# s-a-malik/fumi

Hardware: AMD Instinct MI355X
Metric: episodes/sec (5-way 5-shot FuMI) (higher is better)
Workload: dtype f32; 1 GPU; FuMI 5-way 5-shot, 32 query/class, ResNet-152-style 2048-d embeddings, im_hid [256,64], GloVe-300 token text (L=128, V=20000, mean pool), text_hid 256, 1 inner step, second-order meta-gradient + Adam step; BASELINE.json configs[1]; episodes_per_gpu=32, global_meta_batch=32, parallelism=episode-sharded x1, 1 all-reduce of the flat gradient

## Files before the change

### fumi_amd/csrc/common.h

```cpp
#pragma once
#include <hip/hip_runtime.h>
#include <stdint.h>
#include <stddef.h>
#include <vector>
#include "../../include/fumi_hip.h"

typedef float f32x4 __attribute__((ext_vector_type(4)));
typedef float f32x16 __attribute__((ext_vector_type(16)));

struct f32pair { float x, y; };
struct ProfRec { int phase; hipEvent_t a, b; };
struct fumi_ws {
    int device;
    char* base;
    size_t cap;
    size_t off;
    int* status;
    int* status_host;
    const float* pub_src; float* pub_dst; int pub_n; unsigned long long pub_seq;
    struct AdamPending* adam;
    struct GlovePending* glove;
    float* text_grad;
    int* acnt;
    int* hcnt;
// ... 498 lines not shown
    if (tid < parts * N) {
        const int part = tid / N, n = tid - part * N;
        float s0 = 0.f, s1 = 0.f;
        int m = part;
        for (; m + parts < M; m += 2 * parts) { s0 += X[(long)m * ld + n]; s1 += X[(long)(m + parts) * ld + n]; }
        if (m < M) s0 += X[(long)m * ld + n];
        lds[part * N + n] = s0 + s1;
    }
    __syncthreads();
    for (int n = tid; n < N; n += nt) {
        float s = 0.f;
        for (int pp = 0; pp < parts; ++pp) s += lds[pp * N + n];
        f(n, s);
    }
}
__host__ __device__ __forceinline__ int wg_ld(int cols) { return ((cols + 31) & ~31) + 4; }

__device__ __forceinline__ void wg_stage_tab_to_lds(StageTab* Tl, int ntab = 1, int kernarg_bytes = 0) {
    const int* src = (const int*)__builtin_amdgcn_kernarg_segment_ptr();
    int* dst = (int*)Tl;
    for (int i = threadIdx.x; i < ntab * (int)(sizeof(StageTab) / 4); i += blockDim.x) dst[i] = src[i];
    if (kernarg_bytes > 0) {
        const int first = ntab * (int)sizeof(StageTab) / 64, last = (kernarg_bytes + 63) / 64;
        const int ln = first + (int)threadIdx.x;
        if (ln < last) {
            int dummy;
            asm volatile("global_load_dword %0, %1, off" : "=v"(dummy) : "v"((const char*)src + (long)ln * 64) : "memory");
            asm volatile("s_waitcnt vmcnt(0)" ::: "memory");
            asm volatile("" :: "v"(dummy));
        }
    }
// ... 257 lines not shown
```

### fumi_amd/csrc/episode.hip

```cpp
#include "common.h"
#include <algorithm>
#include <stdlib.h>

namespace {

unsigned long long* g_epi_trace = nullptr;
int g_spin_limit = 1 << 22;
constexpr int QR = 32;
constexpr int MAXL = FUMI_MAX_HIDDEN;

struct EpiBuf {
    float *A0, *G;
    float *D, *cs;
    float *bcur[MAXL], *bh;
    float *Wslot[MAXL], *Whslot;
    float *ta[MAXL], *tdz[MAXL], *tp, *te;
    float *lg;
    float *aq[MAXL], *zq[MAXL], *lbar, *qcs;
    float *pW[MAXL], *pb[MAXL], *pWh, *pbh, *pb0, *pD, *ploss, *pcorr;
    float *Wb[MAXL], *bb[MAXL], *Whb, *bhb, *b0b, *Db;
    float *abar[MAXL], *X0, *X1, *eb, *lb;
    float *A0bar;
    float *A0bar_q; int ldsr, ldq;
    float *apart; int *acnt;
// ... 23 lines not shown
    return drop_mix(h + 0xC2B2AE35U * (unsigned)layer);
}
__device__ __forceinline__ float drop_relu(const EpiDims& d, unsigned key, long idx, float z) {
    if (z <= 0.f) return 0.f;
    if (d.drop_thr == 0) return z;
    return drop_mix(key ^ (unsigned)idx) >= d.drop_thr ? z * d.mscale : 0.f;
}
__device__ __forceinline__ f32x4 drop_relu4(const EpiDims& d, unsigned key, long idx, const f32x4& z) {
    f32x4 o;
#pragma unroll
    for (int e = 0; e < 4; ++e) o[e] = drop_relu(d, key, idx + e, z[e]);
    return o;
}
constexpr int QUERY_CALL = 1 << 20;

struct EpiParams {
    const float* W[MAXL];
    const float* b[MAXL];
};

__device__ __forceinline__ int label(const int64_t* y, long i, int N, int* status) {
    long v = y[i];
    if (v < 0 || v >= N) { atomicOr(status, FUMI_ST_LABEL_RANGE); v = 0; }
    return (int)v;
}

__global__ __launch_bounds__(512) void adapt_kernel(EpiDims d, EpiBuf w, EpiParams prm, const int64_t* y_s,
                                                     const float* head, int* status) {
    extern __shared__ __attribute__((aligned(16))) float sm[];
    const int sm_cap = w.lds_adapt;
// ... 103 lines not shown
            wg_mm2(sm, sm_cap, hi, hp, S, dz(i), 1, hi, a(i - 1), hp, 1, [&](int m, int n) { return Wci[(long)m * hp + n]; },
                   [&](int m, int n, float acc, float pre) { Wni[(long)m * hp + n] = pre - alpha * acc; });
            float* bi = w.bcur[i] + (long)b * hi;
            wg_colsum(sm, sm_cap, S, hi, dz(i), hi, [&](int n, float s) { bi[n] -= alpha * s; });
        }
        if (L == 1) __syncthreads();
        {
            wg_ew((long)S * h0, D, D, dz(0), nullptr, [&](long, float x, float y, float) { return x + y; });
        }
        __syncthreads(); STAMP()
    }
    wg_colsum(sm, sm_cap, S, h0, D, h0, [&](int n, float s) { cs[n] = s; });
#undef STAMP
}

__host__ __device__ inline int q_r4(int x) { return (x + 3) & ~3; }
__host__ __device__ inline int q_r16(int x) { return (x + 15) & ~15; }
constexpr int ALDS_CAP = 40000;
struct ALay { int a[MAXL], dz[MAXL], W[MAXL], bi[MAXL], Wh, G, D, e, cs, bh, total; };
__host__ __device__ inline void adapt_layout(ALay& y, int L, const int* h, int S, int N) {
    int off = 0;
    const int RS = q_r4(S);
    for (int i = 0; i < MAXL; ++i) { y.a[i] = y.dz[i] = y.W[i] = y.bi[i] = 0; }
    for (int i = 0; i < L; ++i) { y.a[i] = off; off += RS * wg_ld(h[i]); }
    for (int i = 1; i < L; ++i) { y.dz[i] = off; off += RS * wg_ld(h[i]); }
    y.G = off; off += RS * wg_ld(S);
    y.e = off; off += RS * wg_ld(N);
    y.D = off; off += RS * wg_ld(h[0]);
    for (int i = 1; i < L; ++i) { y.W[i] = off; off += q_r16(h[i]) * wg_ld(h[i - 1]); y.bi[i] = off; off += q_r4(h[i]); }
    y.Wh = off; off += q_r16(N) * wg_ld(h[L - 1]);
    y.cs = off; off += q_r4(h[0]);
    y.bh = off; off += q_r4(N);
// ... 371 lines not shown
               [&](int m, int n, float acc, float pre) { zp[(long)m * hp + n] = pre > 0.f ? acc * d.mscale : 0.f; });
        __syncthreads();
    }
    float* A0bq = w.A0bar_q + ((long)b * w.ldq + r0) * h0;
    wg_copy(A0bq, z(0), (long)nr * h0);
    float* pb0 = w.pb0 + pt * h0;
    wg_colsum(sm, sm_cap, nr, h0, z(0), h0, [&](int n, float s) { pb0[n] = s; });
    __syncthreads();
    float* pD = w.pD + pt * (long)S * h0;
    wg_mm2(sm, sm_cap, S, h0, nr, Gqs, 1, S, z(0), h0, 1, [&](int m, int n) { return pb0[n]; },
           [&](int m, int n, float acc, float pre) { pD[(long)m * h0 + n] = -alpha * (acc + pre); });
}

constexpr int QLDS_CAP = 40000;
struct QLay { int a[MAXL], W[MAXL], bi[MAXL], Wh, Wh2, Gq, D, lq, b0, cs, pb0, bh, total; };
__host__ __device__ inline void query_layout(QLay& y, int L, const int* h, int S, int N, bool fused = false) {
    int off = 0;
    for (int i = 0; i < MAXL; ++i) { y.a[i] = y.W[i] = y.bi[i] = 0; }
    for (int i = 0; i < L; ++i) { y.a[i] = off; off += QR * wg_ld(h[i]); }
    for (int i = 1; i < L; ++i) { y.W[i] = off; off += q_r16(h[i]) * wg_ld(h[i - 1]); y.bi[i] = off; off += q_r4(h[i]); }
    y.Wh = off; off += q_r16(N) * wg_ld(h[L - 1]);
    y.Wh2 = off; if (fused) off += q_r16(N) * wg_ld(h[L - 1]);
    y.Gq = off; off += QR * wg_ld(S);
    y.D = off; off += q_r4(S) * wg_ld(h[0]);
    y.lq = off; off += QR * wg_ld(N);
    y.b0 = off; off += q_r4(h[0]);
    y.cs = off; off += q_r4(h[0]);
    y.pb0 = off; off += q_r4(h[0]);
    y.bh = off; off += q_r4(N);
    y.total = off;
}

template <bool FUSED>
__global__ __launch_bounds__(512) void query_lds_kernel(StageTab stg, StageTab stg_sup, EpiDims d, EpiBuf w, QLay y, const int64_t* y_q,
                                                        float* logits_q, int64_t* preds_q, float* preds_f, int* status,
                                                        const int64_t* y_s) {
    extern __shared__ __attribute__((aligned(16))) float sm[];
    __shared__ float s_loss[QR];
    __shared__ float s_corr[QR];
    __shared__ StageTab s_stg2[2];
    __shared__ int s_lab[QR];
    StageTab& s_stg = s_stg2[0];
    const int tile = blockIdx.x, b = blockIdx.y, tid = threadIdx.x, nt = blockDim.x;
    int qi = 0;
#define QSTAMP() if (w.trace && tid == 0 && blockIdx.x == 0 && blockIdx.y == 0) w.trace[64 + qi++] = __builtin_amdgcn_s_memrealtime();
    QSTAMP()
    const int S = d.S, N = d.N, L = d.L, H = d.H, h0 = d.h[0], Qn = d.Qn;
    const int r0 = tile * QR, nr = min(QR, Qn - r0);
    const float alpha = d.alpha;
    const int ldq = wg_ld(N), ldG = wg_ld(S), ld0 = wg_ld(h0), ldH = wg_ld(H);
    auto a = [&](int i) { return sm + y.a[i]; };
    auto lda = [&](int i) { return wg_ld(d.h[i]); };

    const int my_label = tid < nr ? label(y_q + (long)b * Qn + r0, tid, N, status) : 0;
    const int my_label_s = (FUSED && tid < S) ? label(y_s + (long)b * S, tid, N, status) : 0;
    if (FUSED && tid < S && tid < QR) s_lab[tid] = my_label_s;
    wg_stage_tab_to_lds(s_stg2, 2, (int)(2 * sizeof(StageTab) + sizeof(EpiDims) + sizeof(EpiBuf) + sizeof(QLay) + 64));
    for (int i = tid * 4, tot = y.total; i < tot; i += nt * 4) *(f32x4*)(sm + i) = (f32x4){0.f, 0.f, 0.f, 0.f};
    __syncthreads(); QSTAMP()
    int whq = y.Wh;
    if constexpr (FUSED) {
        const int nt_ = (Qn + QR - 1) / QR;
        const bool lead = tile == 0 && d.taped;
        const bool lead_w = tile == (nt_ > 1 ? 1 : 0) && d.taped, lead_r = tile == (nt_ > 2 ? 2 : 0) && d.taped;
        const f32x4 z4s = {0.f, 0.f, 0.f, 0.f};
        f32x4 qv[4]; bool qok[4];
        {
            const float* A0q = w.A0 + ((long)b * (S + Qn) + S + r0) * h0;
            const int c4n = h0 >> 2;
#pragma unroll
            for (int i = 0; i < 4; ++i) {
                const int f = tid + 512 * i, m = f / c4n, n = (f - m * c4n) << 2;
                qok[i] = m < nr;
                qv[i] = *(const f32x4*)(A0q + (long)(qok[i] ? m : 0) * h0 + (qok[i] ? n : 0));
            }
        }
        wg_stage_rows<20>(&s_stg2[1], b, tile, 0, nr, sm);
        wg_lds_barrier();
        float* a0 = a(0); float* a1 = a(1); float* W1 = sm + y.W[1]; float* b1 = sm + y.bi[1];
        float* Wh = sm + y.Wh; float* Wh2 = sm + y.Wh2; float* bh = sm + y.bh; float* Dl = sm + y.D; float* csl = sm + y.cs;
        const float* b0l = sm + y.b0; float* e_ = sm + y.lq;
        const int h1 = d.h[1], ld1 = wg_ld(h1);
        const long tp = (long)b * w.ntape;
        auto store_img = [&](float* dst, long drs, const float* img, int ld, int rows, int cols) {
            const int c4n = (cols + 3) >> 2;
            for (int i = tid; i < rows * c4n; i += nt) {
                const int r = i / c4n, cc = (i - r * c4n) << 2;
                wg_st4(dst + (long)r * drs + cc, *(const f32x4*)(img + r * ld + cc), min(4, cols - cc));
            }
        };
        if (lead_w) {
            store_img(w.Wslot[1] + (long)b * w.nslot * ((long)h1 * h0), h0, W1, ld0, h1, h0);
            store_img(w.Whslot + (long)b * w.nslot * N * H, H, Wh, ldH, N, H);
        }
        {
            const unsigned key0 = drop_key(d, b, 0, 0);
            float* ta0 = w.ta[0] + tp * S * h0;
// ... 98 lines not shown
        wg_lds_barrier(); QSTAMP()
    }

    {
        float* a0 = a(0);
        const float* b0l = sm + y.b0; const float* csl = sm + y.cs;
        const unsigned keyq0 = drop_key(d, b, QUERY_CALL, 0);
        wg_lmm_wide<true>(nr, h0, S, sm + y.Gq, ldG, sm + y.D, ld0, [&](int m, int n, const f32x4& acc, int, auto) {
            float* p = a0 + m * ld0 + n;
            const f32x4 pre = *(const f32x4*)p + (*(const f32x4*)(b0l + n) - alpha * *(const f32x4*)(csl + n));
            *(f32x4*)p = drop_relu4(d, keyq0, (long)(r0 + m) * h0 + n, pre - alpha * acc);
        });
    }
    wg_lds_barrier(); QSTAMP()
    for (int i = 1; i < L; ++i) {
        const int hi = d.h[i], hp = d.h[i - 1];
        float* ai = a(i); const int ldi = lda(i);
        const float* bi = sm + y.bi[i];
        const unsigned keyqi = drop_key(d, b, QUERY_CALL, i);
        wg_lmm<true, true>(nr, hi, hp, a(i - 1), lda(i - 1), sm + y.W[i], wg_ld(hp), [&](int m, int n, const f32x4& acc, int) {
            *(f32x4*)(ai + m * ldi + n) = drop_relu4(d, keyqi, (long)(r0 + m) * hi + n, acc + *(const f32x4*)(bi + n));
        });
        wg_lds_barrier(); QSTAMP()
    }
    float* lq = sm + y.lq;
    {
        float* lg = logits_q + ((long)b * Qn + r0) * N;
        const float* bhl = sm + y.bh;
        wg_lmm<true, true>(nr, N, H, a(L - 1), ldH, sm + whq, ldH, [&](int m, int n, const f32x4& acc, int cnt) {
            const f32x4 v = acc + *(const f32x4*)(bhl + n);
            *(f32x4*)(lq + m * ldq + n) = v;
// ... 41 lines not shown
            wg_st4(pWh + m * H + n, acc, cnt);
        });
        float* pbh = w.pbh + pt * N;
        wg_lcolsum(nr, N, lbar, ldq, [&](int n, float s) { pbh[n] = s; });
    }
    wg_lds_barrier(); QSTAMP()
    {
        float* zl = a(L - 1);
        wg_lmm_wide<true>(nr, H, N, lbar, ldq, sm + whq, ldH, [&](int m, int n, const f32x4& acc, int, auto) {
            float* p = zl + m * ldH + n;
            *(f32x4*)p = relu_bwd4(*(const f32x4*)p, acc);
        });
    }
    wg_lds_barrier(); QSTAMP()
    for (int i = L - 1; i >= 1; --i) {
        const int hi = d.h[i], hp = d.h[i - 1];
        const float* zi = a(i); const int ldi = lda(i), ldp = lda(i - 1);
        float* pWi = w.pW[i] + pt * (long)hi * hp;
        wg_lmm_wide<false>(hi, hp, nr, zi, ldi, a(i - 1), ldp, [&](int m, int n, const f32x4& acc, int cnt, auto) {
            wg_st4(pWi + (long)m * hp + n, acc, cnt);
        });
        float* pbi = w.pb[i] + pt * hi;
        wg_lcolsum(nr, hi, zi, ldi, [&](int n, float s) { pbi[n] = s; });
        wg_lds_barrier(); QSTAMP()
        float* zp = a(i - 1);
        wg_lmm_wide<true>(nr, hp, hi, zi, ldi, sm + y.W[i], wg_ld(hp), [&](int m, int n, const f32x4& acc, int, auto) {
            float* p = zp + m * ldp + n;
            *(f32x4*)p = relu_bwd4(*(const f32x4*)p, acc);
        });
        wg_lds_barrier(); QSTAMP()
    }
// ... 154 lines not shown
                   [&](int m, int n) { return f32pair{Db[(long)m * h0 + n], cs[n]}; },
                   [&](int m, int n, float acc, f32pair pre) { Db[(long)m * h0 + n] = pre.x - alpha * (acc + pre.y); });
            __syncthreads();
        }
    }
    float* hb = head_bar + (long)b * N * (H + 1);
    for (int j = tid; j < N * H; j += nt) hb[(j / H) * (H + 1) + (j % H)] = Whb[j];
    for (int j = tid; j < N; j += nt) hb[j * (H + 1) + H] = bhb[j];
}

constexpr int RLDS_CAP = 40000;
struct RLay {
    int Wb[MAXL], bb[MAXL], a[MAXL], dz[MAXL], W[MAXL], ab[MAXL];
    int Db, A0bs, b0b, Whb, bhb, Wh, p, e, eb, G, dab0, X0, X1, cs, ldX, total;
};
inline void reverse_layout(RLay& y, int L, const int* h, int S, int N, int P) {
    int off = 0;
    const int RS = q_r4(S), h0c = h[0] / P, H = h[L - 1];
    auto take = [&](int rows, int ld) { const int o = off; off += rows * ld; return o; };
    for (int i = 0; i < MAXL; ++i) y.Wb[i] = y.bb[i] = y.a[i] = y.dz[i] = y.W[i] = y.ab[i] = 0;
    int maxh1 = 4;
    for (int i = 1; i < L; ++i) maxh1 = h[i] > maxh1 ? h[i] : maxh1;
    y.ldX = wg_ld(maxh1);
    for (int i = 1; i < L; ++i) {
        const int kc = i == 1 ? h0c : h[i - 1];
        y.Wb[i] = take(q_r16(h[i]), wg_ld(kc)); y.W[i] = take(q_r16(h[i]), wg_ld(kc)); y.bb[i] = take(1, q_r4(h[i]));
        y.a[i] = take(RS, wg_ld(h[i])); y.dz[i] = take(RS, wg_ld(h[i])); y.ab[i] = take(RS, wg_ld(h[i]));
    }
    y.a[0] = take(RS, wg_ld(h0c)); y.ab[0] = take(RS, wg_ld(h0c)); y.dab0 = take(RS, wg_ld(h0c));
    y.Db = take(RS, wg_ld(h0c)); y.A0bs = take(RS, wg_ld(h0c));
    y.X0 = take(RS, y.ldX); y.X1 = take(RS, y.ldX);
    y.Whb = take(q_r16(N), wg_ld(H)); y.Wh = take(q_r16(N), wg_ld(H));
    y.p = take(RS, wg_ld(N)); y.e = take(RS, wg_ld(N)); y.eb = take(RS, wg_ld(N)); y.G = take(RS, wg_ld(S));
    y.b0b = take(1, q_r4(h0c)); y.cs = take(1, q_r4(h0c)); y.bhb = take(1, q_r4(N));
    y.total = off + 64;
}

__global__ __launch_bounds__(512) void reverse_lds_kernel(StageTab stg_init, StageTab stg_step, EpiDims d, EpiBuf w, RLay y,
                                                          int P, float* loss_b, float* acc_b, float* head_bar) {
    extern __shared__ __attribute__((aligned(16))) float sm[];
    __shared__ StageTab s_stg[2];
    const int tid = threadIdx.x, nt = blockDim.x;
    const int xcd = blockIdx.x & 7, jq = blockIdx.x >> 3;
    const int b = xcd + 8 * (jq / P), c = jq % P;
    if (b >= d.B) return;
    int ri = 0;
#define RSTAMP() if (w.trace && tid == 0 && blockIdx.x == 0) w.trace[128 + ri++] = __builtin_amdgcn_s_memrealtime();
    RSTAMP()
    const int S = d.S, N = d.N, L = d.L, H = d.H, h0 = d.h[0], h0c = h0 / P, c0 = c * h0c, h1 = d.h[1];
    const float alpha = d.alpha, ms = d.mscale;
    const int ntile = w.ntile;
    if (tid == 0 && c == 0) {
        float ls = 0.f, cr = 0.f;
        for (int t = 0; t < ntile; ++t) { ls += w.ploss[(long)b * ntile + t]; cr += w.pcorr[(long)b * ntile + t]; }
        loss_b[b] = ls / (float)d.Qn;
        acc_b[b] = cr / (float)d.Qn;
    }
    if (!d.need_grad) return;

    const int ldc = wg_ld(h0c), ldN = wg_ld(N), ldS = wg_ld(S), ldH = wg_ld(H), ldX = y.ldX;
    auto ldh = [&](int i) { return wg_ld(d.h[i]); };
    const f32x4 z4 = {0.f, 0.f, 0.f, 0.f};
    auto relu_bwd4 = [&](const f32x4& act, const f32x4& g) {
        f32x4 o;
#pragma unroll
        for (int e = 0; e < 4; ++e) o[e] = act[e] > 0.f ? g[e] * ms : 0.f;
        return o;
    };
    auto ew = [&](int cols, auto&& f) {
        const int c4n = (cols + 3) >> 2;
        for (int i = tid; i < S * c4n; i += nt) { const int m = i / c4n; f(m, (i - m * c4n) << 2); }
    };
    auto store_img = [&](float* dst, long drs, const float* img, int ld, int rows, int cols) {
        const int c4n = (cols + 3) >> 2;
        for (int i = tid; i < rows * c4n; i += nt) {
            const int r = i / c4n, cc = (i - r * c4n) << 2;
// ... 6 lines not shown
    __syncthreads(); RSTAMP()
    wg_stage_rows<3, 8>(&s_stg[0], b, 0, c, 0, sm);
    wg_lds_barrier(); RSTAMP()

    float* Wb1 = sm + y.Wb[1]; float* Db = sm + y.Db; float* A0bs = sm + y.A0bs; float* b0b = sm + y.b0b;
    float* Whb = sm + y.Whb; float* bhb = sm + y.bhb; float* cs = sm + y.cs;
    float* a0 = sm + y.a[0]; float* ab0 = sm + y.ab[0]; float* dab0 = sm + y.dab0; float* W1 = sm + y.W[1];
    float* Wh = sm + y.Wh; float* pp = sm + y.p; float* ee = sm + y.e; float* eb = sm + y.eb; float* G = sm + y.G;
    float* Xa = sm + y.X0; float* Xb = sm + y.X1;

    if (d.second_order) {
        for (int t = d.T - 1; t >= 0; --t) {
            const int round = d.T - 1 - t;
            wg_stage_rows<8, 1>(&s_stg[1], b, t, c, 0, sm);
            wg_lds_barrier(); RSTAMP()
            for (int i = 1; i < L; ++i) { float* abi = sm + y.ab[i]; const int ldi = ldh(i); ew(d.h[i], [&](int m, int n) { *(f32x4*)(abi + m * ldi + n) = z4; }); }
            ew(h0c, [&](int m, int n) {
                *(f32x4*)(ab0 + m * ldc + n) = z4;
                *(f32x4*)(dab0 + m * ldc + n) = relu_bwd4(*(const f32x4*)(a0 + m * ldc + n), *(const f32x4*)(Db + m * ldc + n));
            });
            wg_lds_barrier(); RSTAMP()
            const float* dz1 = sm + y.dz[1]; const int ld1 = ldh(1);
            wg_lmm<true, true>(S, h1, h0c, dab0, ldc, W1, ldc, [&](int m, int n, const f32x4& acc, int) { *(f32x4*)(Xa + m * ldX + n) = acc; });
            wg_lmm<true, true>(S, h1, h0c, a0, ldc, Wb1, ldc, [&](int m, int n, const f32x4& acc, int) {
                float* px = Xa + m * ldX + n; *(f32x4*)px = *(const f32x4*)px - alpha * acc;
            });
            wg_lmm_wide<true>(S, h0c, h1, dz1, ld1, Wb1, ldc, [&](int m, int n, const f32x4& acc, int, auto) {
                float* pa = ab0 + m * ldc + n; *(f32x4*)pa = *(const f32x4*)pa - alpha * acc;
            });
            wg_lds_barrier(); RSTAMP()
            float* xb = w.xpart + (((long)b * 2 + (round & 1)) * 8) * (long)S * h1;
// ... 30 lines not shown
                for (int i = tid; i < S * w4; i += nt) {
                    const int m = i / w4, n = i - m * w4;
                    float v = 0.f;
                    if (n < h1) {
                        if (P > 1) { for (int cc = 0; cc < P; ++cc) v += __hip_atomic_load(xb + (long)cc * S * h1 + m * h1 + n, __ATOMIC_RELAXED, __HIP_MEMORY_SCOPE_AGENT); }
                        else v = Xa[m * ldX + n];
                        v = a1[m * ld1 + n] > 0.f ? (v - alpha * bb1[n]) * ms : 0.f;
                    }
                    Xb[m * ldX + n] = v;
                }
            }
            wg_lds_barrier(); RSTAMP()
            int cur = 1;
            auto X = [&](int i) { return i ? Xb : Xa; };
            for (int i = 2; i < L; ++i) {
                const int hi = d.h[i], hp = d.h[i - 1], ldi = ldh(i), ldp = ldh(i - 1);
                const float* dab = X(cur); float* nxt = X(cur ^ 1);
                const float* bbi = sm + y.bb[i]; float* Wbi = sm + y.Wb[i]; const float* ai = sm + y.a[i];
                const float* dzi = sm + y.dz[i]; float* abp = sm + y.ab[i - 1];
                wg_lmm<true, true>(S, hi, hp, dab, ldX, sm + y.W[i], ldp, [&](int m, int n, const f32x4& acc, int) {
                    *(f32x4*)(nxt + m * ldX + n) = acc - alpha * *(const f32x4*)(bbi + n);
                });
                wg_lmm<true, true>(S, hi, hp, sm + y.a[i - 1], ldp, Wbi, ldp, [&](int m, int n, const f32x4& acc, int) {
                    float* px = nxt + m * ldX + n;
                    *(f32x4*)px = relu_bwd4(*(const f32x4*)(ai + m * ldi + n), *(const f32x4*)px - alpha * acc);
                });
                wg_lmm_wide<true>(S, hp, hi, dzi, ldi, Wbi, ldp, [&](int m, int n, const f32x4& acc, int, auto) {
                    float* pa = abp + m * ldp + n; *(f32x4*)pa = *(const f32x4*)pa - alpha * acc;
                });
                wg_lds_barrier();
                wg_lmm_wide<false>(hi, hp, S, dzi, ldi, dab, ldX, [&](int m, int n, const f32x4& acc, int, auto) {
// ... 24 lines not shown
                    for (int n = 0; n < N; ++n) re[n] = rp[n] * (re[n] - dot) / (float)S;
                    for (int n = N; n < q_r4(N); ++n) re[n] = 0.f;
                }
                wg_lds_barrier(); RSTAMP()
                const float* lb = eb;
                wg_lmm_wide<true>(S, H, N, lb, ldN, Wh, ldH, [&](int m, int n, const f32x4& acc, int, auto) {
                    float* pa = abl + m * ldH + n; *(f32x4*)pa = *(const f32x4*)pa + acc;
                });
                wg_lmm_wide<false>(N, H, S, lb, ldN, aL, ldH, [&](int m, int n, const f32x4& acc, int, auto) {
                    float* pw = Whb + m * ldH + n; *(f32x4*)pw = *(const f32x4*)pw + acc;
                });
                wg_lcolsum(S, N, lb, ldN, [&](int n, float s_) { bhb[n] += s_; });
                wg_lds_barrier(); RSTAMP()
            }
            for (int i = L - 1; i >= 1; --i) {
                const int hi = d.h[i], ldi = ldh(i);
                float* zb = sm + y.ab[i]; const float* ai = sm + y.a[i];
                ew(hi, [&](int m, int n) { float* pz = zb + m * ldi + n; *(f32x4*)pz = relu_bwd4(*(const f32x4*)(ai + m * ldi + n), *(const f32x4*)pz); });
                wg_lds_barrier();
                float* bbw = sm + y.bb[i];
                if (i >= 2) {
                    const int hp = d.h[i - 1], ldp = ldh(i - 1);
                    float* abp = sm + y.ab[i - 1]; float* Wbi = sm + y.Wb[i];
                    wg_lmm_wide<true>(S, hp, hi, zb, ldi, sm + y.W[i], ldp, [&](int m, int n, const f32x4& acc, int, auto) {
                        float* pa = abp + m * ldp + n; *(f32x4*)pa = *(const f32x4*)pa + acc;
                    });
                    wg_lmm_wide<false>(hi, hp, S, zb, ldi, sm + y.a[i - 1], ldp, [&](int m, int n, const f32x4& acc, int, auto) {
                        float* pw = Wbi + m * ldp + n; *(f32x4*)pw = *(const f32x4*)pw + acc;
                    });
                } else {
                    wg_lmm_wide<true>(S, h0c, hi, zb, ldi, W1, ldc, [&](int m, int n, const f32x4& acc, int, auto) {
                        float* pa = ab0 + m * ldc + n; *(f32x4*)pa = *(const f32x4*)pa + acc;
                    });
                    wg_lmm_wide<false>(hi, h0c, S, zb, ldi, a0, ldc, [&](int m, int n, const f32x4& acc, int, auto) {
                        float* pw = Wb1 + m * ldc + n; *(f32x4*)pw = *(const f32x4*)pw + acc;
                    });
                }
// ... 9 lines not shown
            wg_lds_barrier();
            wg_lcolsum(S, h0c, ab0, ldc, [&](int n, float s_) { cs[n] = s_; b0b[n] += s_; });
            wg_lds_barrier();
            wg_lmm_wide<true>(S, h0c, S, G, ldS, ab0, ldc, [&](int m, int n, const f32x4& acc, int, auto) {
                float* pd = Db + m * ldc + n; *(f32x4*)pd = *(const f32x4*)pd - alpha * (acc + *(const f32x4*)(cs + n));
            });
            wg_lds_barrier(); RSTAMP()
        }
    }
    store_img(w.Wb[1] + (long)b * h1 * h0 + c0, h0, Wb1, ldc, h1, h0c);
    store_img(w.A0bar + (long)b * w.ldsr * h0 + c0, h0, A0bs, ldc, S, h0c);
    for (int n = tid; n < h0c; n += nt) w.b0b[(long)b * h0 + c0 + n] = b0b[n];
    if (c == 0) {
        for (int i = 1; i < L; ++i) {
            const float* bbi = sm + y.bb[i];
            for (int n = tid; n < d.h[i]; n += nt) w.bb[i][(long)b * d.h[i] + n] = bbi[n];
            if (i >= 2) store_img(w.Wb[i] + (long)b * d.h[i] * d.h[i - 1], d.h[i - 1], sm + y.Wb[i], ldh(i - 1), d.h[i], d.h[i - 1]);
        }
        float* hb = head_bar + (long)b * N * (H + 1);
        for (int j = tid; j < N * H; j += nt) { const int n = j / H, k = j - n * H; hb[n * (H + 1) + k] = Whb[n * ldH + k]; }
        for (int j = tid; j < N; j += nt) hb[j * (H + 1) + H] = bhb[j];
    }
    RSTAMP()
#undef RSTAMP
}

__global__ void class_text_select_kernel(int N, int S, int Dt, const float* text_s, const int64_t* y_s, float* out,
                                         int* status) {
    const int b = blockIdx.y, n = blockIdx.x, lane = threadIdx.x;
    const int64_t* ys = y_s + (long)b * S;
    int first = S;
    for (int s0 = 0; s0 < S && first == S; s0 += 64) {
// ... 26 lines not shown
}

__global__ void relu_mask_mul_kernel(long n, const float* u, float* g, float scale) {
    for (long i = blockIdx.x * (long)blockDim.x + threadIdx.x; i < n; i += (long)gridDim.x * blockDim.x)
        g[i] = u[i] > 0.f ? g[i] * scale : 0.f;
}

__global__ void split_head_grad_kernel(int B, int N, int H, const float* head_bar, float scale, float* gW, float* gb) {
    const int j = blockIdx.x * blockDim.x + threadIdx.x;
    if (j >= N * (H + 1)) return;
    float s = 0.f;
    for (int b = 0; b < B; ++b) s += head_bar[(long)b * N * (H + 1) + j];
    const int n = j / (H + 1), c = j % (H + 1);
    if (c < H) gW[n * H + c] = scale * s; else gb[n] = scale * s;
}

inline int blocks_for(long n) { long b = (n + 255) / 256; return (int)(b > 2048 ? 2048 : (b < 1 ? 1 : b)); }

struct Carver {
    fumi_ws* ws; size_t bytes;
    float* take(size_t n) {
        bytes += ws_align(n * sizeof(float));
        return ws ? ws_f(ws, n) : nullptr;
    }
};

void carve(Carver& c, const EpisodeProblem& p, EpiBuf& w) {
    const size_t B = p.B, S = p.S, Qn = p.Qn, N = p.N, L = p.L, h0 = p.h[0], H = p.h[L - 1];
    const bool taped = p.need_grad && p.second_order && p.T > 0;
    w.nslot = taped ? p.T + 1 : 1;
// ... 52 lines not shown
    }
}


}

void set_xpanel_trace(void* p);
void set_rn12_trace(void* p);
extern "C" int fumi_hip_set_trace_buffer(int which, void* p) {
    if (which == 0) g_epi_trace = (unsigned long long*)p;
    else if (which == 1) set_xpanel_trace(p);
    else if (which == 2) set_rn12_trace(p);
    else return FUMI_EINVAL;
    return FUMI_OK;
}
extern "C" int fumi_hip_set_spin_limit(int polls) { const int old = g_spin_limit; g_spin_limit = polls < 0 ? 0 : polls; return old; }

size_t episode_workspace_bytes(const EpisodeProblem& p) {
    Carver c{nullptr, 0};
    EpiBuf w;
    w.trace = nullptr;
    carve(c, p, w);
    if (p.need_grad) {
        int kc;
        size_t ns = (size_t)xpanel_bwd_nsplit(p.B, p.S, p.Qn, p.D, p.h[0], &kc);
        if (xpanel_bwd_two_part_ok(p.D, p.h[0])) {
            int nsq, kcq, nss, kcs;
            xpanel_bwd_two_part_split(p.B, p.S, p.Qn, p.D, p.h[0], &nsq, &kcq, &nss, &kcs);
            ns = std::max(ns, (size_t)(nsq + nss));
        }
// ... 37 lines not shown
    if (p.inputs_ready) HIP_TRY(hipEventRecord(p.inputs_ready, st));
    {
        ProfScope ps(ws, st, FUMI_PH_XPANEL_FWD);
        int rider_done = 0;
        if ((rc = launch_xpanel_fwd(st, p.B, p.S, p.Qn, p.D, h0, p.x_s, p.x_q, p.W[0], w.A0, w.G, p.rows.table ? &p.rows : nullptr,
                                    p.fwd_rider, &rider_done, nullptr, nullptr, xpanel_planes(ws, p.B, p.S, p.D, h0), p.glove))) return rc;
        if (p.fwd_rider && !rider_done && p.fwd_rider_fallback && (rc = p.fwd_rider_fallback(p.hook_ctx))) return rc;
    }
    if (p.after_xpanel_fwd && (rc = p.after_xpanel_fwd(p.hook_ctx))) return rc;
    if (p.head_ready) HIP_TRY(hipStreamWaitEvent(st, p.head_ready, 0));
    EpiParams prm;
    for (int i = 0; i < MAXL; ++i) { prm.W[i] = i < p.L ? p.W[i] : nullptr; prm.b[i] = i < p.L ? p.b[i] : nullptr; }
    static const int fuse_env = getenv("FUMI_EPI_FUSE") ? atoi(getenv("FUMI_EPI_FUSE")) : 1;
    QLay qlf; StageTab tbq, tbs;
    bool fuse_q = fuse_env && !getenv("FUMI_EPI_GLOBAL") && p.T == 1 && p.L == 2 && p.S <= QR && (h0 & 3) == 0 && p.head != nullptr;
    if (fuse_q) {
        query_layout(qlf, p.L, p.h, p.S, p.N, true);
        fuse_q = qlf.total <= QLDS_CAP;
    }
    if (fuse_q) {
        const long R = p.S + p.Qn, S = p.S, N = p.N, H = d.H;
        const int h1 = p.h[1];
        tbs.init(); tbq.init();
        tbs.add(w.A0, R * h0, 0, 0, h0, p.S, p.S, h0, qlf.a[0], wg_ld(h0));
        tbs.add(p.W[1], 0, 0, 0, h0, h1, h1, h0, qlf.W[1], wg_ld(h0));
        tbs.add(p.b[1], 0, 0, 0, h1, 1, 1, h1, qlf.bi[1], h1);
        tbs.add(p.head, N * (H + 1), 0, 0, H + 1, p.N, p.N, (int)H, qlf.Wh, wg_ld((int)H));
        tbs.add(p.head + H, N * (H + 1), 0, 0, H + 1, p.N, p.N, 1, qlf.bh, 1);
        tbs.add(p.b[0], 0, 0, 0, h0, 1, 1, h0, qlf.b0, h0);
        tbs.add(w.G + S * S, R * S, (long)QR * S, 0, S, -1, QR, p.S, qlf.Gq, wg_ld(p.S));
        fuse_q = !tbs.bad && tbs.nunits <= 64 * 8 && h0 <= 256;
    }
    if (!fuse_q) {
        ProfScope ps(ws, st, FUMI_PH_ADAPT);
        static const bool force_global_a = getenv("FUMI_EPI_GLOBAL") != nullptr;
        static const int ap_env = getenv("FUMI_ADAPT_P") ? atoi(getenv("FUMI_ADAPT_P")) : 1;
        int AP = 1;
        if (ap_env > 1 && p.L >= 2 && w.acnt && p.B <= FUMI_ACNT) {
            AP = ap_env > 8 ? 8 : ap_env;
            while (AP > 1 && (h0 % (64 * AP) != 0)) AP >>= 1;
        }
        int hs[MAXL];
        for (int i = 0; i < MAXL; ++i) hs[i] = i < p.L ? p.h[i] : 0;
        hs[0] = h0 / AP;
        ALay al; adapt_layout(al, p.L, hs, p.S, p.N);
        const int H = d.H;
// ... 12 lines not shown
            tb.add(p.head + H, N * (H + 1), 0, 0, H + 1, p.N, p.N, 1, al.bh, 1);
            lds_form = !tb.bad && tb.nunits <= 64 * 8;
        }
        if (lds_form) {
            FUMI_SET_DYN_LDS(adapt_lds_kernel, al.total * 4);
            const unsigned grid = AP > 1 ? 8u * ((p.B + 7) / 8) * AP : (unsigned)p.B;
            hipLaunchKernelGGL(adapt_lds_kernel, dim3(grid), dim3(512), al.total * 4, st, tb, d, w, al, prm, p.y_s, ws->status, AP);
        } else {
            FUMI_SET_DYN_LDS(adapt_kernel, w.lds_adapt * 4);
            hipLaunchKernelGGL(adapt_kernel, dim3(p.B), dim3(512), w.lds_adapt * 4, st, d, w, prm, p.y_s, p.head, ws->status);
        }
        LAUNCH_CHECK();
    }
    if (fuse_q) {
        ProfScope ps(ws, st, FUMI_PH_QUERY);
        FUMI_SET_DYN_LDS(query_lds_kernel<true>, qlf.total * 4);
        hipLaunchKernelGGL(query_lds_kernel<true>, dim3(w.ntile, p.B), dim3(512), qlf.total * 4, st, tbq, tbs, d, w, qlf, p.y_q,
                           p.logits_q, p.preds_q, p.preds_f, ws->status, p.y_s);
        LAUNCH_CHECK();
    } else {
        ProfScope ps(ws, st, FUMI_PH_QUERY);
        QLay ql; query_layout(ql, p.L, p.h, p.S, p.N);
        static const bool force_global = getenv("FUMI_EPI_GLOBAL") != nullptr;
        bool lds_form = ql.total <= QLDS_CAP && 7 + 2 * (p.L - 1) <= WG_MAXJOB && !force_global;
        StageTab tb; tb.init();
        if (lds_form) {
            const long R = p.S + p.Qn, S = p.S, N = p.N, H = d.H;
            const long slot = d.taped ? p.T : 0;
            tb.add(w.A0 + S * h0, R * h0, (long)QR * h0, 0, h0, -1, QR, h0, ql.a[0], wg_ld(h0));
            tb.add(w.D, S * h0, 0, 0, h0, p.S, p.S, h0, ql.D, wg_ld(h0));
            for (int i = 1; i < p.L; ++i) {
                const long sz = (long)p.h[i] * p.h[i - 1];
                tb.add(w.Wslot[i] + slot * sz, w.nslot * sz, 0, 0, p.h[i - 1], p.h[i], p.h[i], p.h[i - 1], ql.W[i], wg_ld(p.h[i - 1]));
            }
// ... 28 lines not shown
        HIP_TRY(hipEventRecord(ws->evx[1], ws->side));
    }
    {
        ProfScope ps(ws, st, FUMI_PH_REVERSE);
        static const bool force_global_r = getenv("FUMI_EPI_GLOBAL") != nullptr;
        bool lds_form = p.L >= 2 && p.L <= 4 && w.ntile <= 8 && !force_global_r;
        int P = 0; RLay rl; StageTab ti, tsx;
        if (lds_form) {
            for (int cand = 1; cand <= 8 && !P; cand *= 2) {
                if (h0 % (4 * cand)) break;
                reverse_layout(rl, p.L, p.h, p.S, p.N, cand);
                if (rl.total <= RLDS_CAP) P = cand;
            }
            lds_form = P > 0;
        }
        if (lds_form) {
            const long S = p.S, N = p.N, H = d.H, R = p.S + p.Qn, nt = w.ntile, h0c = h0 / P, h1 = p.h[1];
            ti.init(); tsx.init();
            ti.add(w.pW[1], nt * h1 * h0, 0, h0c, h0, (int)h1, (int)h1, (int)h0c, rl.Wb[1], wg_ld((int)h0c), (int)nt, h1 * h0);
            ti.add(w.pD, nt * S * h0, 0, h0c, h0, p.S, p.S, (int)h0c, rl.Db, wg_ld((int)h0c), (int)nt, S * h0);
            ti.add(w.pb0, nt * h0, 0, h0c, h0, 1, 1, (int)h0c, rl.b0b, (int)h0c, (int)nt, h0);
            ti.add(w.pWh, nt * N * H, 0, 0, H, p.N, p.N, (int)H, rl.Whb, wg_ld((int)H), (int)nt, N * H);
            ti.add(w.pbh, nt * N, 0, 0, N, 1, 1, p.N, rl.bhb, p.N, (int)nt, N);
            for (int i = 1; i < p.L; ++i) {
                const long hi = p.h[i], hp = p.h[i - 1];
                ti.add(w.pb[i], nt * hi, 0, 0, hi, 1, 1, (int)hi, rl.bb[i], (int)hi, (int)nt, hi);
                if (i >= 2) ti.add(w.pW[i], nt * hi * hp, 0, 0, hp, (int)hi, (int)hi, (int)hp, rl.Wb[i], wg_ld((int)hp), (int)nt, hi * hp);
            }
            ti.add(w.G, R * S, 0, 0, S, p.S, p.S, p.S, rl.G, wg_ld(p.S));
            tsx.add(w.ta[0], w.ntape * S * h0, S * h0, h0c, h0, p.S, p.S, (int)h0c, rl.a[0], wg_ld((int)h0c));
            tsx.add(w.Wslot[1], w.nslot * h1 * h0, h1 * h0, h0c, h0, (int)h1, (int)h1, (int)h0c, rl.W[1], wg_ld((int)h0c));
            for (int i = 1; i < p.L; ++i) {
                const long hi = p.h[i], hp = p.h[i - 1];
                tsx.add(w.ta[i], w.ntape * S * hi, S * hi, 0, hi, p.S, p.S, (int)hi, rl.a[i], wg_ld((int)hi));
                tsx.add(w.tdz[i], w.ntape * S * hi, S * hi, 0, hi, p.S, p.S, (int)hi, rl.dz[i], wg_ld((int)hi));
                if (i >= 2) tsx.add(w.Wslot[i], w.nslot * hi * hp, hi * hp, 0, hp, (int)hi, (int)hi, (int)hp, rl.W[i], wg_ld((int)hp));
            }
            tsx.add(w.Whslot, w.nslot * N * H, N * H, 0, H, p.N, p.N, (int)H, rl.Wh, wg_ld((int)H));
            tsx.add(w.tp, w.ntape * S * N, S * N, 0, N, p.S, p.S, p.N, rl.p, wg_ld(p.N));
            tsx.add(w.te, w.ntape * S * N, S * N, 0, N, p.S, p.S, p.N, rl.e, wg_ld(p.N));
            lds_form = !ti.bad && !tsx.bad && ti.nunits <= 64 * 8 && tsx.nunits <= 64 * 8;
        }
        if (lds_form) {
            FUMI_SET_DYN_LDS(reverse_lds_kernel, rl.total * 4);
            hipLaunchKernelGGL(reverse_lds_kernel, dim3(8 * ((p.B + 7) / 8) * P), dim3(512), rl.total * 4, st, ti, tsx, d, w, rl, P,
                               p.loss_b, p.acc_b, p.head_bar);
        } else {
            FUMI_SET_DYN_LDS(reverse_kernel, w.lds_reverse * 4);
            hipLaunchKernelGGL(reverse_kernel, dim3(p.B), dim3(512), w.lds_reverse * 4, st, d, w, p.loss_b, p.acc_b, p.head_bar);
        }
        LAUNCH_CHECK();
    }
    if (p.after_reverse) HIP_TRY(hipEventRecord(p.after_reverse, st));
    {
        ProfScope pr(ws, st, FUMI_PH_REDUCE);
        ReduceSegs own; own.n = 0; own.scale = p.grad_scale;
        const bool defer = p.defer_reduce && p.need_grad && p.defer_reduce->n + 4 + 2 * p.L <= 24;
        ReduceSegs& sg = defer ? *p.defer_reduce : own;
        if (defer) sg.scale = p.grad_scale;
        if (p.stats) { sg.add(p.loss_b, p.B, 1, 1, p.stats); sg.add(p.acc_b, p.B, 1, 1, p.stats + 1); }
        if (p.need_grad) {
// ... 59 lines not shown
```

Baseline: 143,500 episodes/s.

## Add fixed-shape specialized query and reverse kernels for reference FuMI dims

Adds template specializations of the fused query kernel and the LDS reverse kernel that hard-code the reference dimensions (h0=256, h1=64, L=2, T=1, P=4) and the LDS layouts as compile-time constants. Dropout can also be compiled out. In the query kernel, the generic table-driven row staging is replaced by direct unrolled vector loads into LDS. The aim is to cut runtime index arithmetic, kernarg and table staging, and loop overhead on the hot path. The host selects these variants only when the problem shape matches and pointers are 16-byte aligned, so other shapes keep using the generic kernels at the cost of extra code.

Result: faster. 159,200 episodes/s, median of 6 (+11.0%).

```diff
diff --git a/fumi_amd/csrc/common.h b/fumi_amd/csrc/common.h
--- a/fumi_amd/csrc/common.h
+++ b/fumi_amd/csrc/common.h
@@ -536,7 +536,7 @@
         f(n, s);
     }
 }
-__host__ __device__ __forceinline__ int wg_ld(int cols) { return ((cols + 31) & ~31) + 4; }
+__host__ __device__ __forceinline__ constexpr int wg_ld(int cols) { return ((cols + 31) & ~31) + 4; }
 
 __device__ __forceinline__ void wg_stage_tab_to_lds(StageTab* Tl, int ntab = 1, int kernarg_bytes = 0) {
     const int* src = (const int*)__builtin_amdgcn_kernarg_segment_ptr();
diff --git a/fumi_amd/csrc/episode.hip b/fumi_amd/csrc/episode.hip
--- a/fumi_amd/csrc/episode.hip
+++ b/fumi_amd/csrc/episode.hip
@@ -61,6 +61,16 @@
 }
 constexpr int QUERY_CALL = 1 << 20;
 
+constexpr int REF_SP = 32, REF_SQ = 28, REF_NP = 8, REF_H0 = 256, REF_H1 = 64, REF_P = 4;
+template <bool FIX, bool DROP>
+__device__ __forceinline__ void fix_dims(EpiDims& d) {
+    if constexpr (FIX) {
+        d.L = 2; d.T = 1; d.H = REF_H1;
+        d.need_grad = 1; d.second_order = 1; d.taped = 1;
+        if constexpr (!DROP) { d.drop_thr = 0; d.mscale = 1.f; }
+    }
+}
+
 struct EpiParams {
     const float* W[MAXL];
     const float* b[MAXL];
@@ -194,8 +204,8 @@
 #undef STAMP
 }
 
-__host__ __device__ inline int q_r4(int x) { return (x + 3) & ~3; }
-__host__ __device__ inline int q_r16(int x) { return (x + 15) & ~15; }
+__host__ __device__ constexpr int q_r4(int x) { return (x + 3) & ~3; }
+__host__ __device__ constexpr int q_r16(int x) { return (x + 15) & ~15; }
 constexpr int ALDS_CAP = 40000;
 struct ALay { int a[MAXL], dz[MAXL], W[MAXL], bi[MAXL], Wh, G, D, e, cs, bh, total; };
 __host__ __device__ inline void adapt_layout(ALay& y, int L, const int* h, int S, int N) {
@@ -597,7 +607,7 @@
 
 constexpr int QLDS_CAP = 40000;
 struct QLay { int a[MAXL], W[MAXL], bi[MAXL], Wh, Wh2, Gq, D, lq, b0, cs, pb0, bh, total; };
-__host__ __device__ inline void query_layout(QLay& y, int L, const int* h, int S, int N, bool fused = false) {
+__host__ __device__ constexpr void query_layout(QLay& y, int L, const int* h, int S, int N, bool fused = false) {
     int off = 0;
     for (int i = 0; i < MAXL; ++i) { y.a[i] = y.W[i] = y.bi[i] = 0; }
     for (int i = 0; i < L; ++i) { y.a[i] = off; off += QR * wg_ld(h[i]); }
@@ -613,11 +623,19 @@
     y.bh = off; off += q_r4(N);
     y.total = off;
 }
-
-template <bool FUSED>
-__global__ __launch_bounds__(512) void query_lds_kernel(StageTab stg, StageTab stg_sup, EpiDims d, EpiBuf w, QLay y, const int64_t* y_q,
+constexpr QLay ref_qlay() { QLay y{}; const int h[MAXL] = {REF_H0, REF_H1}; query_layout(y, 2, h, REF_SQ, REF_NP, true); return y; }
+
+template <bool FUSED, bool FIX = false, bool DROP = true>
+__global__ __launch_bounds__(512) void query_lds_kernel(StageTab stg, StageTab stg_sup, EpiDims d_arg, EpiBuf w, QLay y_arg, const int64_t* y_q,
                                                         float* logits_q, int64_t* preds_q, float* preds_f, int* status,
                                                         const int64_t* y_s) {
+    static_assert(!FIX || FUSED, "the fixed-shape form is the fused one-step form");
+    EpiDims d_fix = d_arg; fix_dims<FIX, DROP>(d_fix);
+    const EpiDims& d = FIX ? d_fix : d_arg;
+    auto dh = [&](int i) { return FIX ? (i == 0 ? REF_H0 : REF_H1) : d_arg.h[i]; };
+    QLay y_fix = y_arg;
+    if constexpr (FIX) { constexpr QLay k = ref_qlay(); y_fix = k; }
+    const QLay& y = FIX ? y_fix : y_arg;
     extern __shared__ __attribute__((aligned(16))) float sm[];
     __shared__ float s_loss[QR];
     __shared__ float s_corr[QR];
@@ -628,17 +646,17 @@
     int qi = 0;
 #define QSTAMP() if (w.trace && tid == 0 && blockIdx.x == 0 && blockIdx.y == 0) w.trace[64 + qi++] = __builtin_amdgcn_s_memrealtime();
     QSTAMP()
-    const int S = d.S, N = d.N, L = d.L, H = d.H, h0 = d.h[0], Qn = d.Qn;
+    const int S = d.S, N = d.N, L = d.L, H = d.H, h0 = dh(0), Qn = d.Qn;
     const int r0 = tile * QR, nr = min(QR, Qn - r0);
     const float alpha = d.alpha;
     const int ldq = wg_ld(N), ldG = wg_ld(S), ld0 = wg_ld(h0), ldH = wg_ld(H);
     auto a = [&](int i) { return sm + y.a[i]; };
-    auto lda = [&](int i) { return wg_ld(d.h[i]); };
+    auto lda = [&](int i) { return wg_ld(dh(i)); };
 
     const int my_label = tid < nr ? label(y_q + (long)b * Qn + r0, tid, N, status) : 0;
     const int my_label_s = (FUSED && tid < S) ? label(y_s + (long)b * S, tid, N, status) : 0;
     if (FUSED && tid < S && tid < QR) s_lab[tid] = my_label_s;
-    wg_stage_tab_to_lds(s_stg2, 2, (int)(2 * sizeof(StageTab) + sizeof(EpiDims) + sizeof(EpiBuf) + sizeof(QLay) + 64));
+    wg_stage_tab_to_lds(s_stg2, FIX ? 0 : 2, (int)(2 * sizeof(StageTab) + sizeof(EpiDims) + sizeof(EpiBuf) + sizeof(QLay) + 64));
     for (int i = tid * 4, tot = y.total; i < tot; i += nt * 4) *(f32x4*)(sm + i) = (f32x4){0.f, 0.f, 0.f, 0.f};
     __syncthreads(); QSTAMP()
     int whq = y.Wh;
@@ -658,12 +676,48 @@
                 qv[i] = *(const f32x4*)(A0q + (long)(qok[i] ? m : 0) * h0 + (qok[i] ? n : 0));
             }
         }
-        wg_stage_rows<20>(&s_stg2[1], b, tile, 0, nr, sm);
+        if constexpr (FIX) {
+            const float* A0s = stg_sup.base[0] + (long)b * (S + Qn) * REF_H0;
+            const float* W1g = stg_sup.base[1]; const float* b1g = stg_sup.base[2];
+            const float* hdg = stg_sup.base[3] + (long)b * N * (REF_H1 + 1); const float* b0g = stg_sup.base[5];
+            const float* Gg = stg_sup.base[6] + ((long)b * (S + Qn) + r0) * S;
+            constexpr int C4 = REF_H0 / 4;
+            f32x4 va[4], vw[8];
+            float vg[2], vh;
+#pragma unroll
+            for (int k = 0; k < 4; ++k) { const int f = tid + 512 * k, m = f / C4; va[k] = *(const f32x4*)(A0s + (long)(m < S ? m : 0) * REF_H0 + 4 * (f % C4)); }
+#pragma unroll
+            for (int k = 0; k < 8; ++k) { const int f = tid + 512 * k; vw[k] = *(const f32x4*)(W1g + (long)f * 4); }
+#pragma unroll
+            for (int k = 0; k < 2; ++k) {
+                const int f = tid + 512 * k, m = f >> 5, c = f & 31;
+                vg[k] = Gg[(m < nr && c < S) ? (long)m * S + c : 0];
+            }
+            {
+                const int m = tid >> 6, c = tid & 63;
+                vh = hdg[m < N ? m * (REF_H1 + 1) + c : 0];
+            }
+            const f32x4 vb0 = *(const f32x4*)(b0g + 4 * (tid & 63));
+            const f32x4 vb1 = *(const f32x4*)(b1g + 4 * (tid & 15));
+            const float vbh = hdg[tid < N ? tid * (REF_H1 + 1) + REF_H1 : 0];
+#pragma unroll
+            for (int k = 0; k < 4; ++k) { const int f = tid + 512 * k, m = f / C4; if (m < S) *(f32x4*)(sm + y.a[0] + m * wg_ld(REF_H0) + 4 * (f % C4)) = va[k]; }
+#pragma unroll
+            for (int k = 0; k < 8; ++k) { const int f = tid + 512 * k; *(f32x4*)(sm + y.W[1] + (f / C4) * wg_ld(REF_H0) + 4 * (f % C4)) = vw[k]; }
+#pragma unroll
+            for (int k = 0; k < 2; ++k) { const int f = tid + 512 * k, m = f >> 5, c = f & 31; if (m < nr && c < S) sm[y.Gq + m * wg_ld(REF_SQ) + c] = vg[k]; }
+            if ((tid >> 6) < N) sm[y.Wh + (tid >> 6) * wg_ld(REF_H1) + (tid & 63)] = vh;
+            if (tid < REF_H0 / 4) *(f32x4*)(sm + y.b0 + 4 * tid) = vb0;
+            if (tid < REF_H1 / 4) *(f32x4*)(sm + y.bi[1] + 4 * tid) = vb1;
+            if (tid < N) sm[y.bh + tid] = vbh;
+        } else {
+            wg_stage_rows<20>(&s_stg2[1], b, tile, 0, nr, sm);
+        }
         wg_lds_barrier();
         float* a0 = a(0); float* a1 = a(1); float* W1 = sm + y.W[1]; float* b1 = sm + y.bi[1];
         float* Wh = sm + y.Wh; float* Wh2 = sm + y.Wh2; float* bh = sm + y.bh; float* Dl = sm + y.D; float* csl = sm + y.cs;
         const float* b0l = sm + y.b0; float* e_ = sm + y.lq;
-        const int h1 = d.h[1], ld1 = wg_ld(h1);
+        const int h1 = dh(1), ld1 = wg_ld(h1);
         const long tp = (long)b * w.ntape;
         auto store_img = [&](float* dst, long drs, const float* img, int ld, int rows, int cols) {
             const int c4n = (cols + 3) >> 2;
@@ -792,7 +846,7 @@
     }
     wg_lds_barrier(); QSTAMP()
     for (int i = 1; i < L; ++i) {
-        const int hi = d.h[i], hp = d.h[i - 1];
+        const int hi = dh(i), hp = dh(i - 1);
         float* ai = a(i); const int ldi = lda(i);
         const float* bi = sm + y.bi[i];
         const unsigned keyqi = drop_key(d, b, QUERY_CALL, i);
@@ -864,7 +918,7 @@
     }
     wg_lds_barrier(); QSTAMP()
     for (int i = L - 1; i >= 1; --i) {
-        const int hi = d.h[i], hp = d.h[i - 1];
+        const int hi = dh(i), hp = dh(i - 1);
         const float* zi = a(i); const int ldi = lda(i), ldp = lda(i - 1);
         float* pWi = w.pW[i] + pt * (long)hi * hp;
         wg_lmm_wide<false>(hi, hp, nr, zi, ldi, a(i - 1), ldp, [&](int m, int n, const f32x4& acc, int cnt, auto) {
@@ -1049,7 +1103,7 @@
     int Wb[MAXL], bb[MAXL], a[MAXL], dz[MAXL], W[MAXL], ab[MAXL];
     int Db, A0bs, b0b, Whb, bhb, Wh, p, e, eb, G, dab0, X0, X1, cs, ldX, total;
 };
-inline void reverse_layout(RLay& y, int L, const int* h, int S, int N, int P) {
+__host__ __device__ constexpr void reverse_layout(RLay& y, int L, const int* h, int S, int N, int P) {
     int off = 0;
     const int RS = q_r4(S), h0c = h[0] / P, H = h[L - 1];
     auto take = [&](int rows, int ld) { const int o = off; off += rows * ld; return o; };
@@ -1070,9 +1124,19 @@
     y.b0b = take(1, q_r4(h0c)); y.cs = take(1, q_r4(h0c)); y.bhb = take(1, q_r4(N));
     y.total = off + 64;
 }
-
-__global__ __launch_bounds__(512) void reverse_lds_kernel(StageTab stg_init, StageTab stg_step, EpiDims d, EpiBuf w, RLay y,
-                                                          int P, float* loss_b, float* acc_b, float* head_bar) {
+constexpr RLay ref_rlay() { RLay y{}; const int h[MAXL] = {REF_H0, REF_H1}; reverse_layout(y, 2, h, REF_SP, REF_NP, REF_P); return y; }
+static_assert(ref_qlay().total <= QLDS_CAP && ref_rlay().total <= RLDS_CAP, "the reference layouts fit the CU's LDS");
+
+template <bool FIX = false, bool DROP = true>
+__global__ __launch_bounds__(512) void reverse_lds_kernel(StageTab stg_init, StageTab stg_step, EpiDims d_arg, EpiBuf w, RLay y_arg,
+                                                          int P_arg, float* loss_b, float* acc_b, float* head_bar) {
+    EpiDims d_fix = d_arg; fix_dims<FIX, DROP>(d_fix);
+    const EpiDims& d = FIX ? d_fix : d_arg;
+    auto dh = [&](int i) { return FIX ? (i == 0 ? REF_H0 : REF_H1) : d_arg.h[i]; };
+    RLay y_fix = y_arg;
+    if constexpr (FIX) { constexpr RLay k = ref_rlay(); y_fix = k; }
+    const RLay& y = FIX ? y_fix : y_arg;
+    const int P = FIX ? REF_P : P_arg;
     extern __shared__ __attribute__((aligned(16))) float sm[];
     __shared__ StageTab s_stg[2];
     const int tid = threadIdx.x, nt = blockDim.x;
@@ -1082,7 +1146,7 @@
     int ri = 0;
 #define RSTAMP() if (w.trace && tid == 0 && blockIdx.x == 0) w.trace[128 + ri++] = __builtin_amdgcn_s_memrealtime();
     RSTAMP()
-    const int S = d.S, N = d.N, L = d.L, H = d.H, h0 = d.h[0], h0c = h0 / P, c0 = c * h0c, h1 = d.h[1];
+    const int S = d.S, N = d.N, L = d.L, H = d.H, h0 = dh(0), h0c = h0 / P, c0 = c * h0c, h1 = dh(1);
     const float alpha = d.alpha, ms = d.mscale;
     const int ntile = w.ntile;
     if (tid == 0 && c == 0) {
@@ -1094,7 +1158,7 @@
     if (!d.need_grad) return;
 
     const int ldc = wg_ld(h0c), ldN = wg_ld(N), ldS = wg_ld(S), ldH = wg_ld(H), ldX = y.ldX;
-    auto ldh = [&](int i) { return wg_ld(d.h[i]); };
+    auto ldh = [&](int i) { return wg_ld(dh(i)); };
     const f32x4 z4 = {0.f, 0.f, 0.f, 0.f};
     auto relu_bwd4 = [&](const f32x4& act, const f32x4& g) {
         f32x4 o;
@@ -1131,7 +1195,7 @@
             const int round = d.T - 1 - t;
             wg_stage_rows<8, 1>(&s_stg[1], b, t, c, 0, sm);
             wg_lds_barrier(); RSTAMP()
-            for (int i = 1; i < L; ++i) { float* abi = sm + y.ab[i]; const int ldi = ldh(i); ew(d.h[i], [&](int m, int n) { *(f32x4*)(abi + m * ldi + n) = z4; }); }
+            for (int i = 1; i < L; ++i) { float* abi = sm + y.ab[i]; const int ldi = ldh(i); ew(dh(i), [&](int m, int n) { *(f32x4*)(abi + m * ldi + n) = z4; }); }
             ew(h0c, [&](int m, int n) {
                 *(f32x4*)(ab0 + m * ldc + n) = z4;
                 *(f32x4*)(dab0 + m * ldc + n) = relu_bwd4(*(const f32x4*)(a0 + m * ldc + n), *(const f32x4*)(Db + m * ldc + n));
@@ -1192,7 +1256,7 @@
             int cur = 1;
             auto X = [&](int i) { return i ? Xb : Xa; };
             for (int i = 2; i < L; ++i) {
-                const int hi = d.h[i], hp = d.h[i - 1], ldi = ldh(i), ldp = ldh(i - 1);
+                const int hi = dh(i), hp = dh(i - 1), ldi = ldh(i), ldp = ldh(i - 1);
                 const float* dab = X(cur); float* nxt = X(cur ^ 1);
                 const float* bbi = sm + y.bb[i]; float* Wbi = sm + y.Wb[i]; const float* ai = sm + y.a[i];
                 const float* dzi = sm + y.dz[i]; float* abp = sm + y.ab[i - 1];
@@ -1247,13 +1311,13 @@
                 wg_lds_barrier(); RSTAMP()
             }
             for (int i = L - 1; i >= 1; --i) {
-                const int hi = d.h[i], ldi = ldh(i);
+                const int hi = dh(i), ldi = ldh(i);
                 float* zb = sm + y.ab[i]; const float* ai = sm + y.a[i];
                 ew(hi, [&](int m, int n) { float* pz = zb + m * ldi + n; *(f32x4*)pz = relu_bwd4(*(const f32x4*)(ai + m * ldi + n), *(const f32x4*)pz); });
                 wg_lds_barrier();
                 float* bbw = sm + y.bb[i];
                 if (i >= 2) {
-                    const int hp = d.h[i - 1], ldp = ldh(i - 1);
+                    const int hp = dh(i - 1), ldp = ldh(i - 1);
                     float* abp = sm + y.ab[i - 1]; float* Wbi = sm + y.Wb[i];
                     wg_lmm_wide<true>(S, hp, hi, zb, ldi, sm + y.W[i], ldp, [&](int m, int n, const f32x4& acc, int, auto) {
                         float* pa = abp + m * ldp + n; *(f32x4*)pa = *(const f32x4*)pa + acc;
@@ -1293,8 +1357,8 @@
     if (c == 0) {
         for (int i = 1; i < L; ++i) {
             const float* bbi = sm + y.bb[i];
-            for (int n = tid; n < d.h[i]; n += nt) w.bb[i][(long)b * d.h[i] + n] = bbi[n];
-            if (i >= 2) store_img(w.Wb[i] + (long)b * d.h[i] * d.h[i - 1], d.h[i - 1], sm + y.Wb[i], ldh(i - 1), d.h[i], d.h[i - 1]);
+            for (int n = tid; n < dh(i); n += nt) w.bb[i][(long)b * dh(i) + n] = bbi[n];
+            if (i >= 2) store_img(w.Wb[i] + (long)b * dh(i) * dh(i - 1), dh(i - 1), sm + y.Wb[i], ldh(i - 1), dh(i), dh(i - 1));
         }
         float* hb = head_bar + (long)b * N * (H + 1);
         for (int j = tid; j < N * H; j += nt) { const int n = j / H, k = j - n * H; hb[n * (H + 1) + k] = Whb[n * ldH + k]; }
@@ -1351,6 +1415,8 @@
     const int n = j / (H + 1), c = j % (H + 1);
     if (c < H) gW[n * H + c] = scale * s; else gb[n] = scale * s;
 }
+
+template <auto K> struct KernTag { static constexpr auto fn = K; };
 
 inline int blocks_for(long n) { long b = (n + 255) / 256; return (int)(b > 2048 ? 2048 : (b < 1 ? 1 : b)); }
 
@@ -1433,6 +1499,8 @@
     else return FUMI_EINVAL;
     return FUMI_OK;
 }
+static int g_epi_fixed_last = 0;
+extern "C" int fumi_hip_epi_fixed_last() { return g_epi_fixed_last; }
 extern "C" int fumi_hip_set_spin_limit(int polls) { const int old = g_spin_limit; g_spin_limit = polls < 0 ? 0 : polls; return old; }
 
 size_t episode_workspace_bytes(const EpisodeProblem& p) {
@@ -1500,8 +1568,15 @@
     static const int fuse_env = getenv("FUMI_EPI_FUSE") ? atoi(getenv("FUMI_EPI_FUSE")) : 1;
     QLay qlf; StageTab tbq, tbs;
     bool fuse_q = fuse_env && !getenv("FUMI_EPI_GLOBAL") && p.T == 1 && p.L == 2 && p.S <= QR && (h0 & 3) == 0 && p.head != nullptr;
+    static const int fixed_env = getenv("FUMI_EPI_FIXED") ? atoi(getenv("FUMI_EPI_FIXED")) : 1;
+    const bool fixed = fixed_env && !getenv("FUMI_EPI_GLOBAL") && p.T == 1 && p.L == 2 && p.h[0] == REF_H0 && p.h[1] == REF_H1 &&
+                       p.S <= REF_SP && p.N <= REF_NP && p.need_grad && p.second_order;
+    bool fixed_q = fixed && fuse_q && p.S <= REF_SQ;
+    g_epi_fixed_last = 0;
+    const bool drop = d.drop_thr != 0;
     if (fuse_q) {
-        query_layout(qlf, p.L, p.h, p.S, p.N, true);
+        if (fixed_q) qlf = ref_qlay();
+        else query_layout(qlf, p.L, p.h, p.S, p.N, true);
         fuse_q = qlf.total <= QLDS_CAP;
     }
     if (fuse_q) {
@@ -1516,6 +1591,8 @@
         tbs.add(p.b[0], 0, 0, 0, h0, 1, 1, h0, qlf.b0, h0);
         tbs.add(w.G + S * S, R * S, (long)QR * S, 0, S, -1, QR, p.S, qlf.Gq, wg_ld(p.S));
         fuse_q = !tbs.bad && tbs.nunits <= 64 * 8 && h0 <= 256;
+        auto a16 = [](const void* q) { return (((uintptr_t)q) & 15) == 0; };
+        fixed_q = fixed_q && a16(p.W[1]) && a16(p.b[1]) && a16(p.b[0]);
     }
     if (!fuse_q) {
         ProfScope ps(ws, st, FUMI_PH_ADAPT);
@@ -1558,10 +1635,18 @@
     }
     if (fuse_q) {
         ProfScope ps(ws, st, FUMI_PH_QUERY);
-        FUMI_SET_DYN_LDS(query_lds_kernel<true>, qlf.total * 4);
-        hipLaunchKernelGGL(query_lds_kernel<true>, dim3(w.ntile, p.B), dim3(512), qlf.total * 4, st, tbq, tbs, d, w, qlf, p.y_q,
-                           p.logits_q, p.preds_q, p.preds_f, ws->status, p.y_s);
-        LAUNCH_CHECK();
+        auto launch = [&](auto tag) -> int {
+            constexpr auto kern = decltype(tag)::fn;
+            FUMI_SET_DYN_LDS(kern, qlf.total * 4);
+            hipLaunchKernelGGL(kern, dim3(w.ntile, p.B), dim3(512), qlf.total * 4, st, tbq, tbs, d, w, qlf, p.y_q,
+                               p.logits_q, p.preds_q, p.preds_f, ws->status, p.y_s);
+            LAUNCH_CHECK();
+            return FUMI_OK;
+        };
+        if (fixed_q) g_epi_fixed_last |= 1;
+        if (fixed_q) rc = drop ? launch(KernTag<query_lds_kernel<true, true, true>>{}) : launch(KernTag<query_lds_kernel<true, true, false>>{});
+        else rc = launch(KernTag<query_lds_kernel<true>>{});
+        if (rc) return rc;
     } else {
         ProfScope ps(ws, st, FUMI_PH_QUERY);
         QLay ql; query_layout(ql, p.L, p.h, p.S, p.N);
@@ -1620,6 +1705,8 @@
             }
             lds_form = P > 0;
         }
+        const bool fixed_r = fixed && lds_form && P == REF_P;
+        if (fixed_r) rl = ref_rlay();
         if (lds_form) {
             const long S = p.S, N = p.N, H = d.H, R = p.S + p.Qn, nt = w.ntile, h0c = h0 / P, h1 = p.h[1];
             ti.init(); tsx.init();
@@ -1648,9 +1735,18 @@
             lds_form = !ti.bad && !tsx.bad && ti.nunits <= 64 * 8 && tsx.nunits <= 64 * 8;
         }
         if (lds_form) {
-            FUMI_SET_DYN_LDS(reverse_lds_kernel, rl.total * 4);
-            hipLaunchKernelGGL(reverse_lds_kernel, dim3(8 * ((p.B + 7) / 8) * P), dim3(512), rl.total * 4, st, ti, tsx, d, w, rl, P,
-                               p.loss_b, p.acc_b, p.head_bar);
+            auto launch = [&](auto tag) -> int {
+                constexpr auto kern = decltype(tag)::fn;
+                FUMI_SET_DYN_LDS(kern, rl.total * 4);
+                hipLaunchKernelGGL(kern, dim3(8 * ((p.B + 7) / 8) * P), dim3(512), rl.total * 4, st, ti, tsx, d, w, rl, P,
+                                   p.loss_b, p.acc_b, p.head_bar);
+                LAUNCH_CHECK();
+                return FUMI_OK;
+            };
+            if (fixed_r) g_epi_fixed_last |= 2;
+            if (fixed_r) rc = drop ? launch(KernTag<reverse_lds_kernel<true, true>>{}) : launch(KernTag<reverse_lds_kernel<true, false>>{});
+            else rc = launch(KernTag<reverse_lds_kernel<>>{});
+            if (rc) return rc;
         } else {
             FUMI_SET_DYN_LDS(reverse_kernel, w.lds_reverse * 4);
             hipLaunchKernelGGL(reverse_kernel, dim3(p.B), dim3(512), w.lds_reverse * 4, st, d, w, p.loss_b, p.acc_b, p.head_bar);
```
